# MarSaKi/VLN-BEVBert

Measured on AMD Instinct MI355X. Metric: pretrain_samples_per_sec, higher is better.
Workload: dtype bf16+fp32-residual

## Files before the change

### vln_bevbert_amd/arena.py

```python
import math

import torch

from . import lib
from .lib import ptr, stream


def call(name, *args):
    from . import ops
    return ops.call(name, *args)

CHUNK = 1024
_ZERO_KERNEL = __import__("os").environ.get("BEVBERT_ZERO_KERNEL", "0") == "1"
NO_DECAY = ("bias", "LayerNorm.bias", "LayerNorm.weight")


def _round_up(n, m):
    return (n + m - 1) // m * m


class ParamArena:
    _serial = 0

    def __init__(self, module, device, compute_dtype=torch.float32, groups=()):
        self.device = torch.device(device)
        self.compute_dtype = compute_dtype
        named = [(n, p) for n, p in module.named_parameters()]
        by_name = dict(named)
        in_group = {}
        for gi, g in enumerate(groups):
            for n in g:
                in_group[n] = gi
        layout, seen_groups = [], set()
        for n, p in named:
            if n in in_group:
                gi = in_group[n]
                if gi in seen_groups:
                    continue
                seen_groups.add(gi)
                layout.append(list(groups[gi]))
            else:
                layout.append([n])
        self.slices = {}
        off = 0
        seg_meta = []
        for seg in layout:
            start = off
            decays = set()
            for n in seg:
                k = by_name[n].numel()
                self.slices[n] = (off, k)
                off += k
                decays.add(not any(nd in n for nd in NO_DECAY))
            assert len(decays) == 1, f"group {seg} mixes weight-decay classes"
            off = _round_up(off, CHUNK)
            seg_meta.append((start, off, decays.pop(), seg))
        self.numel = off
        self.n_params = sum(p.numel() for _, p in named)
        dev = self.device
        self.params = torch.zeros(off, dtype=torch.float32, device=dev)
        self.grads = torch.zeros(off, dtype=torch.float32, device=dev)
        self.exp_avg = None
        self.exp_avg_sq = None
        self.shadow = torch.zeros(off, dtype=compute_dtype, device=dev) if compute_dtype != torch.float32 else None
        self._flags_host = torch.zeros(off // CHUNK, dtype=torch.uint8)
        self._seg_of = {}
        for start, end, decay, seg in seg_meta:
            if decay:
                self._flags_host[start // CHUNK:end // CHUNK] |= 1
            for n in seg:
                self._seg_of[n] = (start // CHUNK, end // CHUNK)
        self.flags = self._flags_host.to(dev)
        self.chunk_steps = torch.zeros(off // CHUNK, dtype=torch.int32, device=dev)
        self._touched = set()
        self._flags_dirty = False
        self.publish_grads = True
        self.allreduce_group = None
        self.defer_allreduce = False
        self._cb_queued = False
        self._fresh = []
        self._published = []
        self._param_versions = None
        self.step_count = 0
        self._scalars = torch.zeros(4, dtype=torch.float32, device=dev)
        self._partials = torch.zeros(1024, dtype=torch.float32, device=dev)
        self.named = named
        for n, p in named:
            o, k = self.slices[n]
            view = self.params[o:o + k].view(p.shape)
            view.copy_(p.data.to(dev, torch.float32))
            p.data = view
            p.main_grad = self.grads[o:o + k].view(p.shape)
            p.compute = self.shadow[o:o + k].view(p.shape) if self.shadow is not None else p.data
            p.arena = self
            p.arena_name = n
        self._index = {n: i for i, (n, _) in enumerate(named)}
        self.fold_store = False
        ParamArena._serial += 1
        self.fold_key = ("arena", ParamArena._serial)
        tables = {id(m.weight) for m in module.modules() if isinstance(m, torch.nn.Embedding)}
        self._fold_ranges = []
        for o, k, _ in sorted((*self.slices[n], n) for n, p in named if p.dim() >= 2 and id(p) not in tables):
            if self._fold_ranges and self._fold_ranges[-1][1] == o:
                self._fold_ranges[-1][1] = o + k
            else:
                self._fold_ranges.append([o, o + k])
        self._fold_starts = [a for a, _ in self._fold_ranges]
        self._fold_comp = {}
        self.sync_shadow()
        self._param_versions = sum(p._version for _, p in named)

    def packed(self, names, shape):
        o0, _ = self.slices[names[0]]
        total = 0
        for n in names:
            o, k = self.slices[n]
            assert o == o0 + total, f"{names} are not contiguous in the arena"
            total += k
        assert total == math.prod(shape)
        src = self.shadow if self.shadow is not None else self.params
        return src[o0:o0 + total].view(shape), self.grads[o0:o0 + total].view(shape)

    def touch(self, param):
        n = param.arena_name
        if n not in self._touched:
            self._touched.add(n)
            a, b = self._seg_of[n]
            self._flags_host[a:b] |= 2
            self._flags_dirty = True
        if self.publish_grads:
            self._note_backward_write(param)

    def _note_backward_write(self, param):
        if not self._cb_queued:
            try:
                torch.autograd.Variable._execution_engine.queue_callback(self._publish)
            except RuntimeError:
                return
            self._cb_queued = True
        self._fresh.append(param)

    def _publish(self):
        self._cb_queued = False
        self.sync()
        if self.device.type == "cuda":
            from . import ops
            ops.RT.scratch.reset()
        fresh = self._fresh
        if self.allreduce_group is not None and not self.defer_allreduce:
            import torch.distributed as dist
            dist.all_reduce(self.grads, group=self.allreduce_group)
            self.grads.div_(dist.get_world_size(self.allreduce_group))
            used = torch.zeros(len(self.named), dtype=torch.int32, device=self.grads.device)
            if fresh:
                used[torch.tensor(sorted({self._index[p.arena_name] for p in fresh}), device=used.device)] = 1
            dist.all_reduce(used, op=dist.ReduceOp.MAX, group=self.allreduce_group)
            mine = {id(p) for p in fresh}
            fresh = list(fresh) + [self.named[i][1] for i in used.nonzero().flatten().tolist()
                                   if id(self.named[i][1]) not in mine]
        for p in fresh:
            if p.grad is None:
                p.grad = p.main_grad
                self._published.append(p)
        self._fresh.clear()

    def maybe_lazy_zero(self):
        if self._published and any(p.grad is None for p in self._published):
            for p in self._published:
                p.grad = None
            self._published.clear()
            self.zero_grad()

    def maybe_refresh_shadow(self):
        if self.shadow is None or not self.publish_grads:
            return
        v = 0
        for _, p in self.named:
            v += p._version
        if v != self._param_versions:
            if self._param_versions is not None:
                self.sync_shadow()
            self._param_versions = v

    def sync_shadow(self):
        if self.shadow is not None:
            call("bevbert_cast_f32", ptr(self.params), ptr(self.shadow), self.numel, lib.dtype_code(self.compute_dtype),
                 stream())

    def sync(self):
        if self.device.type == "cuda":
            from . import ops
            ops.WgradStream.flush_all()
            cur = torch.cuda.current_stream(self.device)
            for side in ops.Branches.side_streams():
                if ops.Branches.enabled or side not in ops.WgradStream.streams or ops.WgradStream.dirty:
                    cur.wait_stream(side)
            ops.WgradStream.dirty = False
            ops.WgradStream.release()

    def store_ok(self, sink_ptr, n):
        import bisect
        off, rem = divmod(sink_ptr - self.grads.data_ptr(), 4)
        if rem or off < 0 or off + n > self.numel:
            return False
        i = bisect.bisect_right(self._fold_starts, off) - 1
        return i >= 0 and off + n <= self._fold_ranges[i][1]

    def _arm_fold(self):
        from . import ops
        ops.ReduceQueue.store_ok = self.store_ok if self.fold_store else None
        ops.ReduceQueue.fold_norm = None

    def _name_at(self, sink_ptr):
        off = (sink_ptr - self.grads.data_ptr()) // 4
        return next((n for n, (o, k) in self.slices.items() if o <= off < o + k), f"arena offset {off}")

    def fold_check_zero(self, stores):
        base = self.grads.data_ptr()
        views = [self.grads[(p - base) // 4:(p - base) // 4 + n] for p, n in stores]
        counts = torch.stack([torch.count_nonzero(v) for v in views]).tolist()
        bad = [(self._name_at(p), c) for (p, _), c in zip(stores, counts) if c]
        if bad:
            raise lib.BevBertHipError(
                "store-mode fold: the gradient of " + ", ".join(f"{n} ({c} non-zero elements)" for n, c in bad[:4])
                + " is not zero before the step's fold -- something other than the split-K fold writes it, or the arena "
                "was not zeroed for this step (BEVBERT_FOLD_STORE=0 turns the store mode off)")

    def _fold_complement(self, entry):
        ent = self._fold_comp.get(id(entry))
        if ent is not None and ent[0] is entry:
            return ent[1:]
        if torch.cuda.is_current_stream_capturing():
            raise lib.BevBertHipError("fold-norm complement table missing during graph capture (warm-up steps build it)")
        import numpy as np
        base, recs, pos = self.grads.data_ptr(), [], 0
        for p, n, _ in sorted(entry["norm_jobs"]) + [(base + 4 * self.numel, 0, 0)]:
            o = (p - base) // 4
            for a in range(pos, o, 16384):
                recs.append((base + 4 * a, (min(a + 16384, o) - a) // 4))
            pos = o + n
            assert pos % 4 == 0, "fold sinks are float4-aligned"
        from . import ops
        if entry["nslots"] + len(recs) > ops.ReduceQueue.SLOT_CAPACITY:
            return None
        t = np.zeros(len(recs), dtype=np.dtype([("ptr", "<u8"), ("n4", "<u4"), ("slot", "<u4")]))
        if recs:
            t["ptr"], t["n4"] = zip(*recs)
        t["slot"] = entry["nslots"] + np.arange(len(recs))
        dev = torch.from_numpy(t.view(np.uint8).copy()).to(self.device)
        if len(self._fold_comp) > 64:
            self._fold_comp.clear()
        self._fold_comp[id(entry)] = (entry, dev, len(recs), 16 * int(t["n4"].sum()))
        return dev, len(recs), 16 * int(t["n4"].sum())

    def _clip_from_fold(self, pre_scale, max_norm):
        from . import ops
        rec, ops.ReduceQueue.fold_norm = ops.ReduceQueue.fold_norm, None
        if rec is None or rec["owner"] is not self:
            return False
        entry = rec["entry"]
        comp = self._fold_complement(entry)
        if comp is None:
            return False
        table, ntasks, _ = comp
        slots = ops.ReduceQueue.register_slots(self.device)
        call("bevbert_sumsq_tasks", table.data_ptr(), ntasks, stream())
        call("bevbert_clip_from_slots", ptr(slots), entry["nslots"] + ntasks, pre_scale, max_norm, ptr(self._scalars),
             stream())
        if entry["fresh"] and not torch.cuda.is_current_stream_capturing():
            entry["fresh"] = False
            self._fold_check_norm(entry, slots, pre_scale)
        return True

    def _fold_check_norm(self, entry, slots, pre_scale):
        want = float(torch.linalg.vector_norm(self.grads, dtype=torch.float64)) * pre_scale
        got = float(self._scalars[0])
        if abs(got - want) <= 1e-5 * want or (got == 0.0 and want == 0.0):
            return
        base, culprit = self.grads.data_ptr(), "a range outside the folds"
        for p, n, s0 in entry["norm_jobs"]:
            o = (p - base) // 4
            w = float(self.grads[o:o + n].double().pow(2).sum())
            g = float(slots[s0:s0 + (n // 4 + 4095) // 4096].double().sum())
            if abs(g - w) > 1e-5 * max(w, 1e-30):
                culprit = self._name_at(p)
                break
        raise lib.BevBertHipError(
            f"fused gradient norm {got!r} differs from the arena's {want!r}: the gradient of {culprit} changed after the "
            "step's fold (BEVBERT_FOLD_STORE=0 turns the fused norm off)")

    def backward_done(self):
        self.sync()

    def zero_grad(self, overlap=False):
        self.sync()
        if self.device.type == "cuda":
            from . import ops
            ops.RT.scratch.reset()
            self._arm_fold()
            if overlap:
                if getattr(self, "_zero_stream", None) is None:
                    from .hwqueues import side_stream
                    self._zero_stream = side_stream(self.device)
                self._zero_stream.wait_stream(torch.cuda.current_stream(self.device))
                with torch.cuda.stream(self._zero_stream):
                    if _ZERO_KERNEL:
                        self.grads.zero_()
                    else:
                        call("bevbert_zero", ptr(self.grads), self.grads.numel() * 4, stream())
                self._zero_pending = True
                return
            call("bevbert_zero", ptr(self.grads), self.grads.numel() * 4, stream())
            return
        self.grads.zero_()

    def wait_zero(self):
        if getattr(self, "_zero_pending", False):
            torch.cuda.current_stream(self.device).wait_stream(self._zero_stream)
            self._zero_pending = False

    def load_state_dict_into(self, module, sd, strict=True):
        out = module.load_state_dict(sd, strict=strict)
        self.sync_shadow()
        return out

    def set_lr(self, lr):
        self._scalars[2:3].fill_(float(lr))
        self._lr_set = True

    def upload_flags(self):
        if self._flags_dirty:
            self.flags.copy_(self._flags_host, non_blocking=True)
            self._flags_dirty = False

    def clip_and_step(self, lr=None, betas=(0.9, 0.98), eps=1e-6, weight_decay=0.01, max_norm=5.0, grad_pre_scale=1.0,
                      fused_norm=False):
        self.sync()
        if self.exp_avg is None:
            self.exp_avg = torch.zeros_like(self.params)
            self.exp_avg_sq = torch.zeros_like(self.params)
        if lr is not None:
            self.set_lr(lr)
        elif not getattr(self, "_lr_set", False):
            raise RuntimeError("clip_and_step(lr=None) reads the device-resident learning rate: call set_lr() first "
                               "(the slot starts at 0, which would silently turn AdamW and its weight decay into a no-op)")
        if not torch.cuda.is_current_stream_capturing():
            self.upload_flags()
        self.step_count += 1
        max_norm = float(max_norm if max_norm is not None else -1.0)
        if not (fused_norm and self._clip_from_fold(float(grad_pre_scale), max_norm)):
            call("bevbert_grad_norm_clip", ptr(self.grads), self.numel, float(grad_pre_scale), max_norm,
                 ptr(self._partials), ptr(self._scalars), stream())
        call("bevbert_adamw_step", ptr(self.params), ptr(self.grads), ptr(self.exp_avg), ptr(self.exp_avg_sq),
             ptr(self.shadow), ptr(self.flags), ptr(self.chunk_steps), self.numel, self._scalars[1:].data_ptr(),
             self._scalars[2:].data_ptr(), 0.0, float(betas[0]), float(betas[1]), float(eps), float(weight_decay),
             stream())

    def grad_norm(self):
        return self._scalars[0]
```

### vln_bevbert_amd/csrc/optimizer.hip

```cpp
#include <math.h>
#include <type_traits>

#include "rowops_common.h"

#define ACCUM_U 4
#define ACCUM_SC 4
template <typename T, bool STORE = false>
__device__ __forceinline__ float accum_fold(const T* part_, float* sink_, size_t stride4, size_t n4, int S, size_t first,
                                            size_t step) {
  const BB_GLOBAL T* __restrict__ part = (const BB_GLOBAL T*)part_;
  BB_GLOBAL float* __restrict__ sink = (BB_GLOBAL float*)sink_;
  float sq = 0.f;
  for (size_t i = first; i < n4; i += ACCUM_U * step) {
    size_t idx[ACCUM_U];
    float4 acc[ACCUM_U];
#pragma unroll
    for (int u = 0; u < ACCUM_U; ++u) {
      idx[u] = i + u * step < n4 ? i + u * step : n4 - 1;
      if constexpr (STORE) acc[u] = make_float4(0.f, 0.f, 0.f, 0.f);
      else acc[u] = gld4<float>(sink + idx[u] * 4);
    }
    int s = 0;
    for (; s + ACCUM_SC <= S; s += ACCUM_SC) {
      float4 v[ACCUM_SC][ACCUM_U];
#pragma unroll
      for (int k = 0; k < ACCUM_SC; ++k)
#pragma unroll
        for (int u = 0; u < ACCUM_U; ++u) v[k][u] = gld4<T>(part + ((size_t)(s + k) * stride4 + idx[u]) * 4);
#pragma unroll
      for (int k = 0; k < ACCUM_SC; ++k)
#pragma unroll
        for (int u = 0; u < ACCUM_U; ++u) add4(acc[u], v[k][u]);
    }
    for (; s < S; ++s) {
      float4 v[ACCUM_U];
#pragma unroll
      for (int u = 0; u < ACCUM_U; ++u) v[u] = gld4<T>(part + ((size_t)s * stride4 + idx[u]) * 4);
#pragma unroll
      for (int u = 0; u < ACCUM_U; ++u) add4(acc[u], v[u]);
    }
#pragma unroll
    for (int u = 0; u < ACCUM_U; ++u)
      if (i + u * step < n4) {
        const bb_f4v o = {acc[u].x, acc[u].y, acc[u].z, acc[u].w};
        *reinterpret_cast<BB_GLOBAL bb_f4v*>(sink + idx[u] * 4) = o;
        sq += (acc[u].x * acc[u].x + acc[u].y * acc[u].y) + (acc[u].z * acc[u].z + acc[u].w * acc[u].w);
      }
  }
  return sq;
}

template <typename T>
__global__ __launch_bounds__(256) void accum_partials_kernel(const T* __restrict__ partials, float* __restrict__ sink,
                                                             int S, size_t n4) {
  accum_fold<T>(partials, sink, n4, n4, S, (size_t)blockIdx.x * 256 + threadIdx.x, (size_t)gridDim.x * 256);
}

struct AccumTask {
  const void* partials;
  float* sink;
  unsigned long long n4_total;
  unsigned int off4, n4;
  int S, dtype;
};
#define ACCUM_STORE 0x100
#define ACCUM_NORM 0x200
__device__ __forceinline__ float block_sum_256(float s) {
  __shared__ float sh[4];
  s = wave_sum(s);
  if ((threadIdx.x & 63) == 0) sh[threadIdx.x >> 6] = s;
  __syncthreads();
  return (sh[0] + sh[1]) + (sh[2] + sh[3]);
}
template <typename T, bool STORE>
__device__ __forceinline__ float accum_task(const AccumTask& t) {
  return accum_fold<T, STORE>((const T*)t.partials + (size_t)t.off4 * 4, t.sink, t.n4_total, t.n4, t.S, threadIdx.x, 256);
}
__global__ __launch_bounds__(256) void multi_accum_kernel(const AccumTask* __restrict__ tasks, float* __restrict__ slots,
                                                          unsigned int capacity) {
  const AccumTask t = tasks[blockIdx.x];
  const bool bf16 = (t.dtype & 0xff) == BB_BF16;
  float sq;
  if (t.dtype & ACCUM_STORE) sq = bf16 ? accum_task<bf16_raw, true>(t) : accum_task<float, true>(t);
  else sq = bf16 ? accum_task<bf16_raw, false>(t) : accum_task<float, false>(t);
  const unsigned int slot = (unsigned int)t.dtype >> 12;
  if ((t.dtype & ACCUM_NORM) && slot < capacity) {
    sq = block_sum_256(sq);
    if (threadIdx.x == 0) slots[slot] = sq;
  }
}

__global__ __launch_bounds__(256) void sumsq_kernel(const float* __restrict__ g, size_t n4, float* __restrict__ partials) {
  float s = 0.f;
  for (size_t i = (size_t)blockIdx.x * 256 + threadIdx.x; i < n4; i += (size_t)gridDim.x * 256) {
    const float4 v = *reinterpret_cast<const float4*>(g + i * 4);
    s += (v.x * v.x + v.y * v.y) + (v.z * v.z + v.w * v.w);
  }
  __shared__ float sh[4];
  s = wave_sum(s);
  if ((threadIdx.x & 63) == 0) sh[threadIdx.x >> 6] = s;
  __syncthreads();
  if (threadIdx.x == 0) partials[blockIdx.x] = (sh[0] + sh[1]) + (sh[2] + sh[3]);
}

struct SumsqTask {
  const float* ptr;
  unsigned int n4, slot;
};
__global__ __launch_bounds__(256) void sumsq_tasks_kernel(const SumsqTask* __restrict__ tasks, float* __restrict__ slots,
                                                          unsigned int capacity) {
  const SumsqTask t = tasks[blockIdx.x];
  if (t.slot >= capacity) return;
  const unsigned int n4 = t.n4 < 4096u ? t.n4 : 4096u;
  float s = 0.f;
  if (n4) {
    const BB_GLOBAL float* __restrict__ g = (const BB_GLOBAL float*)t.ptr;
    float4 v[16];
#pragma unroll
    for (int u = 0; u < 16; ++u) {
      const unsigned int i = threadIdx.x + u * 256;
      v[u] = gld4<float>(g + (size_t)(i < n4 ? i : n4 - 1) * 4);
    }
#pragma unroll
    for (int u = 0; u < 16; ++u)
      if (threadIdx.x + u * 256 < n4) s += (v[u].x * v[u].x + v[u].y * v[u].y) + (v[u].z * v[u].z + v[u].w * v[u].w);
  }
  s = block_sum_256(s);
  if (threadIdx.x == 0) slots[t.slot] = s;
}

__global__ void clip_coef_kernel(const float* __restrict__ partials, int n, float pre_scale, float max_norm,
                                 float* __restrict__ scalars) {
  __shared__ double sh[256];
  double s = 0.0;
  for (int i = threadIdx.x; i < n; i += 256) s += (double)partials[i];
  sh[threadIdx.x] = s;
  __syncthreads();
  for (int o = 128; o > 0; o >>= 1) {
    if (threadIdx.x < o) sh[threadIdx.x] += sh[threadIdx.x + o];
    __syncthreads();
  }
  if (threadIdx.x == 0) {
    const float norm = (float)sqrt(sh[0]) * pre_scale;
    float coef = 1.0f;
    if (max_norm > 0.f) {
      coef = max_norm / (norm + 1e-6f);
      coef = coef < 1.0f ? coef : 1.0f;
    }
    scalars[0] = norm;
    scalars[1] = pre_scale * coef;
  }
}

__global__ __launch_bounds__(256) void adamw_kernel(float* __restrict__ p, const float* __restrict__ g,
                                                    float* __restrict__ m, float* __restrict__ v,
                                                    bf16_raw* __restrict__ p_bf16, const uint8_t* __restrict__ flags,
                                                    int* __restrict__ chunk_steps, size_t nchunks,
                                                    const float* __restrict__ gscale_ptr,
                                                    const float* __restrict__ lr_ptr, float lr, float beta1,
                                                    float beta2, float eps, float wd, float log2_beta1,
                                                    float log2_beta2) {
  if (lr_ptr) lr = *lr_ptr;
  const size_t chunk = blockIdx.x;
  if (chunk >= nchunks) return;
  const uint8_t f = flags[chunk];
  if (!(f & 2)) return;
  const int t = chunk_steps[chunk] + 1;
  __syncthreads();
  if (threadIdx.x == 0) chunk_steps[chunk] = t;
  const float bc1 = 1.0f - __builtin_amdgcn_exp2f((float)t * log2_beta1);
  const float bc2 = 1.0f - __builtin_amdgcn_exp2f((float)t * log2_beta2);
  const float step_size = lr * sqrtf(bc2) / bc1;
  const float gs = gscale_ptr ? *gscale_ptr : 1.0f;
  const float decay = (f & 1) ? lr * wd : 0.f;
  const size_t i = chunk * 1024 + threadIdx.x * 4;
  const float4 gg = *reinterpret_cast<const float4*>(g + i);
  float4 pp = *reinterpret_cast<float4*>(p + i);
  float4 mm = *reinterpret_cast<float4*>(m + i);
  float4 vv = *reinterpret_cast<float4*>(v + i);
#define UPD(c)                                                    \
  {                                                               \
    const float gr = gg.c * gs;                                   \
    mm.c = mm.c * beta1 + (1.0f - beta1) * gr;                    \
    vv.c = vv.c * beta2 + (1.0f - beta2) * gr * gr;               \
    pp.c = pp.c - step_size * (mm.c / (sqrtf(vv.c) + eps));       \
    pp.c = pp.c - decay * pp.c;                                   \
  }
  UPD(x) UPD(y) UPD(z) UPD(w)
#undef UPD
  *reinterpret_cast<float4*>(p + i) = pp;
  *reinterpret_cast<float4*>(m + i) = mm;
  *reinterpret_cast<float4*>(v + i) = vv;
  if (p_bf16 != nullptr) st4<bf16_raw>(p_bf16 + i, pp);
}

template <typename TO>
__global__ __launch_bounds__(256) void cast_f32_kernel(const float* __restrict__ src, TO* __restrict__ dst, size_t n4) {
  for (size_t i = (size_t)blockIdx.x * 256 + threadIdx.x; i < n4; i += (size_t)gridDim.x * 256)
    st4<TO>(dst + i * 4, *reinterpret_cast<const float4*>(src + i * 4));
}

BEVBERT_API int bevbert_accum_partials(const void* partials, float* sink, int S, int64_t n, int dtype,
                                       hipStream_t stream) {
  BB_REQUIRE(n % 4 == 0 && S >= 1, "accum_partials: n must be a multiple of 4 and S >= 1");
  if (n == 0) return BB_OK;
  size_t nb = ((size_t)n / 4 + 255) / 256;
  if (nb > 8192) nb = 8192;
  const bool type_ok = bb_with_type(dtype, [&](auto t) {
    using T = decltype(t);
    hipLaunchKernelGGL(accum_partials_kernel<T>, dim3(nb), dim3(256), 0, stream, (const T*)partials, sink, S, (size_t)n / 4);
  });
  if (!type_ok) return bb_dtype_unsupported("accum_partials", dtype);
  BB_CHECK_LAUNCH("accum_partials");
  return BB_OK;
}

BEVBERT_API int bevbert_multi_accum(const void* tasks, int ntasks, hipStream_t stream) {
  static_assert(sizeof(AccumTask) == 40, "AccumTask is part of the C ABI");
  if (ntasks <= 0) return BB_OK;
  BB_REQUIRE(tasks != nullptr, "multi_accum: null task table");
  int capacity = 0;
  float* slots = bb_fold_norm_slots(&capacity);
  hipLaunchKernelGGL(multi_accum_kernel, dim3(ntasks), dim3(256), 0, stream, (const AccumTask*)tasks, slots,
                     (unsigned int)(slots ? capacity : 0));
  BB_CHECK_LAUNCH("multi_accum");
  return BB_OK;
}

BEVBERT_API int bevbert_sumsq_tasks(const void* tasks, int ntasks, hipStream_t stream) {
  static_assert(sizeof(SumsqTask) == 16, "SumsqTask is part of the C ABI");
  if (ntasks <= 0) return BB_OK;
  int capacity = 0;
  float* slots = bb_fold_norm_slots(&capacity);
  BB_REQUIRE(tasks != nullptr && slots != nullptr, "sumsq_tasks: null task table, or no slot array registered");
  hipLaunchKernelGGL(sumsq_tasks_kernel, dim3(ntasks), dim3(256), 0, stream, (const SumsqTask*)tasks, slots,
                     (unsigned int)capacity);
  BB_CHECK_LAUNCH("sumsq_tasks");
  return BB_OK;
}

BEVBERT_API int bevbert_grad_norm_clip(const float* grads, int64_t n, float pre_scale, float max_norm,
                                       float* partials, float* scalars, hipStream_t stream) {
  BB_REQUIRE(n % 4 == 0, "grad_norm_clip: n must be a multiple of 4");
  hipLaunchKernelGGL(sumsq_kernel, dim3(1024), dim3(256), 0, stream, grads, (size_t)n / 4, partials);
  hipLaunchKernelGGL(clip_coef_kernel, dim3(1), dim3(256), 0, stream, partials, 1024, pre_scale, max_norm, scalars);
  BB_CHECK_LAUNCH("grad_norm_clip");
  return BB_OK;
}

BEVBERT_API int bevbert_clip_from_slots(const float* slots, int n, float pre_scale, float max_norm, float* scalars,
                                        hipStream_t stream) {
  BB_REQUIRE(n >= 0 && (slots != nullptr || n == 0) && scalars != nullptr, "clip_from_slots: null pointer or negative count");
  hipLaunchKernelGGL(clip_coef_kernel, dim3(1), dim3(256), 0, stream, slots, n, pre_scale, max_norm, scalars);
  BB_CHECK_LAUNCH("clip_from_slots");
  return BB_OK;
}

BEVBERT_API int bevbert_adamw_step(float* params, const float* grads, float* exp_avg, float* exp_avg_sq,
                                   void* params_bf16, const uint8_t* chunk_flags, int* chunk_steps, int64_t n,
                                   const float* grad_scale_dev, const float* lr_dev, float lr, float beta1,
                                   float beta2, float eps, float weight_decay, hipStream_t stream) {
  BB_REQUIRE(n % 1024 == 0, "adamw_step: arena length must be a multiple of 1024 elements");
  BB_REQUIRE(chunk_steps != nullptr, "adamw_step: per-chunk step counters are required");
  const size_t nchunks = (size_t)n / 1024;
  hipLaunchKernelGGL(adamw_kernel, dim3(nchunks), dim3(256), 0, stream, params, grads, exp_avg, exp_avg_sq,
                     (bf16_raw*)params_bf16, chunk_flags, chunk_steps, nchunks, grad_scale_dev, lr_dev, lr, beta1, beta2, eps,
                     weight_decay, (float)log2((double)beta1), (float)log2((double)beta2));
  BB_CHECK_LAUNCH("adamw_step");
  return BB_OK;
}

BEVBERT_API int bevbert_cast_f32(const float* src, void* dst, int64_t n, int dst_dtype, hipStream_t stream) {
  BB_REQUIRE(n % 4 == 0, "cast_f32: n must be a multiple of 4");
  if (n == 0) return BB_OK;
  size_t nb = ((size_t)n / 4 + 255) / 256;
  if (nb > 8192) nb = 8192;
  const bool type_ok = bb_with_type_of<bf16_raw, _Float16>(dst_dtype, [&](auto t) {
    using T = decltype(t);
    hipLaunchKernelGGL(cast_f32_kernel<T>, dim3(nb), dim3(256), 0, stream, src, (T*)dst, (size_t)n / 4);
  });
  if (!type_ok) {
    bb_set_error("cast_f32: dst dtype %d unsupported", dst_dtype);
    return BB_EUNSUPPORTED;
  }
  BB_CHECK_LAUNCH("cast_f32");
  return BB_OK;
}
```

### vln_bevbert_amd/train.py

```python
import contextlib
import os
import random

import torch
import torch.distributed as dist

from . import capture, ops
from .static_step import GraphedStep, StaticBatch


def warmup_linear_lr(step, base_lr, warmup_steps, total_steps):
    f = step / warmup_steps if step < warmup_steps else max(0, (total_steps - step) / (total_steps - warmup_steps))
    lr = base_lr * f
    return lr if lr > 0 else 1e-8


def load_gemm_tuning():
    import os
    path = os.path.join(os.path.dirname(os.path.abspath(__file__)), "tunableop_results.csv")
    if os.environ.get("BEVBERT_GEMM_TUNING", "1") != "1" or not os.path.exists(path):
        return 0
    try:
        import torch.cuda.tunable as tunable
        tunable.enable(True)
        tunable.tuning_enable(False)
        tunable.record_untuned_enable(False) if hasattr(tunable, "record_untuned_enable") else None
        tunable.set_filename(path + ".unused")
        ok = tunable.read_file(path)
        return len(tunable.get_results()) if ok else 0
    except Exception:
        return 0


class TaskSampler:

    def __init__(self, task_ratio="mlm.5.sap.5.masksem.1", seed=0):
        parts = task_ratio.split(".")
        self.tasks = parts[::2]
        ratios = [int(r) for r in parts[1::2]]
        self.pool = [t for t, r in zip(self.tasks, ratios) for _ in range(r)]
        self.rng = random.Random(seed)

    def next(self):
        return self.rng.choice(self.pool)


class GradReducer:

    def __init__(self, flat_grads, split, group=None, force=False, exchange=None):
        import os
        self.exchange = exchange or os.environ.get("BEVBERT_GRAD_EXCHANGE", "fp32")
        assert self.exchange in ("fp32", "bf16", "bf16_a2a"), self.exchange
        self.flat = flat_grads
        self.split = int(split)
        self.group = group
        self.world = dist.get_world_size(group) if dist.is_available() and dist.is_initialized() else 1
        self.active = self.world > 1 or (force and dist.is_available() and dist.is_initialized())
        self.cuda = flat_grads.is_cuda
        self.stream = None
        if self.cuda and self.active:
            from .hwqueues import side_stream
            self.stream = side_stream(flat_grads.device)
        self.queue_report = None
        self._works = []
        self._phase_a_done = False
        self._done = []
        self.occupied = None
        self.timeline = None

    _settled = {}

    def settle_collective_queue(self):
        if self.queue_report is not None or not (self.cuda and self.active) or \
                os.environ.get("BEVBERT_COLLECTIVE_QUEUE_CHECK", "1") != "1":
            return self.queue_report
        if dist.get_backend(self.group) != "nccl":
            self.queue_report = {"backend": dist.get_backend(self.group), "checked": False}
            return self.queue_report
        settled = GradReducer._settled.get((self.flat.device.index, id(self.group)))
        if settled is not None:
            self.group, self.queue_report = settled
            return self.queue_report
        key = (self.flat.device.index, id(self.group))
        from .hwqueues import steer_stream_pool
        st = steer_stream_pool(self.flat.device, like=self.stream)
        rep = {"steered": st and {"pool": st["pool"], "next": st["next"], "wanted": sum(st["wanted"])},
               "waits_behind_compute": self.collectives_wait_behind_compute()}
        if rep["waits_behind_compute"] and self.group is None:
            st = steer_stream_pool(self.flat.device, like=self.stream)
            self.group = dist.new_group(backend=dist.get_backend())
            rep["own_group"] = {"steered": st and {"pool": st["pool"], "next": st["next"]},
                                "waits_behind_compute": self.collectives_wait_behind_compute()}
        self.queue_report = rep
        GradReducer._settled[key] = (self.group, rep)
        return rep

    def collectives_wait_behind_compute(self, busy_ms=3.0):
        if not (self.cuda and self.active and self.stream is not None):
            return None
        dev = self.flat.device
        main = torch.cuda.current_stream(dev)
        busy = torch.empty(64 << 20, dtype=torch.float32, device=dev)
        t = torch.zeros(256, device=dev)
        dist.all_reduce(t, group=self.group)
        dist.barrier(group=self.group)
        torch.cuda.synchronize(dev)
        from .hwqueues import pick_copy_stream
        issue = pick_copy_stream(dev)
        m1, c1 = torch.cuda.Event(), torch.cuda.Event()
        for _ in range(max(4, int(busy_ms / 0.06))):
            busy.fill_(1.0)
        m1.record(main)
        with torch.cuda.stream(issue):
            dist.all_reduce(t, group=self.group, async_op=True).wait()
            c1.record(issue)
        while not c1.query():
            pass
        waited = torch.tensor([1.0 if m1.query() else 0.0], device=dev)
        torch.cuda.synchronize(dev)
        dist.all_reduce(waited, op=dist.ReduceOp.MAX, group=self.group)
        return bool(waited.item() > 0)

    def drop_pending(self):
        self._works, self._done, self._phase_a_done = [], [], False

    def launch_region(self, lo, hi):
        lo, hi = max(0, int(lo)), min(int(hi), self.flat.numel())
        if self.active and hi > lo:
            self._launch(lo, hi)
            self._done.append((lo, hi))

    def _remaining(self):
        gaps, at = [], 0
        for lo, hi in sorted(self._done):
            if lo > at:
                gaps.append((at, lo))
            at = max(at, hi)
        if at < self.flat.numel():
            gaps.append((at, self.flat.numel()))
        if self.occupied is not None:
            gaps = [(lo, hi) for lo, hi in gaps if self._holds_a_tensor(lo, hi)]
        return gaps

    def _holds_a_tensor(self, lo, hi):
        if self.occupied is None:
            return True
        import bisect
        i = bisect.bisect_right(self._occ_starts, lo) - 1
        return (i >= 0 and self.occupied[i][1] > lo) or (i + 1 < len(self._occ_starts) and self._occ_starts[i + 1] < hi)

    def set_occupied(self, slices):
        self.occupied = sorted((int(o), int(o) + int(k)) for o, k in slices)
        self._occ_starts = [o for o, _ in self.occupied]

    def _exchange_bf16(self, view):
        W, n = self.world, view.numel()
        per = -(-n // W)
        send = torch.zeros(W * per, dtype=torch.bfloat16, device=view.device)
        send[:n].copy_(view)
        if self.exchange == "bf16":
            mine = torch.empty(per, dtype=torch.bfloat16, device=view.device)
            dist.reduce_scatter_tensor(mine, send, op=dist.ReduceOp.SUM, group=self.group)
            dist.all_gather_into_tensor(send, mine, group=self.group)
        else:
            recv = torch.empty_like(send)
            as_wire = (lambda t: t) if view.is_cuda else (lambda t: t.view(torch.uint8))
            dist.all_to_all_single(as_wire(recv), as_wire(send), group=self.group)
            mine = recv.view(W, per).float().sum(0).to(torch.bfloat16)
            dist.all_gather_into_tensor(as_wire(send), as_wire(mine), group=self.group)
        view.copy_(send[:n])

    def _launch(self, lo, hi):
        if hi <= lo:
            return
        view = self.flat[lo:hi]
        if self.cuda:
            ops.WgradStream.flush_all()
        if self.stream is not None:
            self.stream.wait_stream(torch.cuda.current_stream())
            for side in ops.Branches.side_streams():
                if ops.Branches.enabled or side not in ops.WgradStream.streams or ops.WgradStream.dirty:
                    self.stream.wait_stream(side)
            with torch.cuda.stream(self.stream):
                if self.timeline is not None:
                    e0, e1 = torch.cuda.Event(enable_timing=True), torch.cuda.Event(enable_timing=True)
                    e0.record(self.stream)
                    self.timeline.append((lo, hi, e0, e1))
                if self.exchange != "fp32":
                    self._exchange_bf16(view)
                else:
                    self._works.append(dist.all_reduce(view, op=dist.ReduceOp.SUM, group=self.group, async_op=True))
                if self.timeline is not None:
                    if self._works and self.exchange == "fp32":
                        self._works[-1].wait()
                    e1.record(self.stream)
        elif self.exchange != "fp32":
            self._exchange_bf16(view)
        else:
            self._works.append(dist.all_reduce(view, op=dist.ReduceOp.SUM, group=self.group, async_op=True))

    def launch_uncovered(self, lo, hi):
        for a, b in self._remaining():
            a, b = max(a, int(lo)), min(b, int(hi))
            if b > a and self._holds_a_tensor(a, b):
                self.launch_region(a, b)

    def phase_a(self, *_):
        if self.active and not self._phase_a_done:
            self._phase_a_done = True
            self.launch_uncovered(self.split, self.flat.numel())

    def finish(self):
        if self.active:
            for lo, hi in self._remaining():
                self._launch(lo, hi)
            for w in self._works:
                w.wait()
            if self.stream is not None:
                torch.cuda.current_stream().wait_stream(self.stream)
        self._works = []
        self._phase_a_done = False
        self._done = []


def fold_store_allowed(device_type, reducer_active, early_flush, env=None):
    env = os.environ if env is None else env
    return env.get("BEVBERT_FOLD_STORE", "1") == "1" and device_type == "cuda" and not reducer_active and not early_flush


class PretrainTrainer:
    def __init__(self, model, arena, learning_rate=5e-5, warmup_steps=10000, num_train_steps=100000,
                 betas=(0.9, 0.98), weight_decay=0.01, grad_norm=5.0, seed=0, rank=0, world_size=1, overlap=True,
                 force_collectives=False):
        self.model, self.arena = model, arena
        arena.publish_grads = False
        self.lr, self.warmup, self.total = learning_rate, warmup_steps, num_train_steps
        self.betas, self.wd, self.grad_norm = betas, weight_decay, grad_norm
        self.seed, self.rank, self.world = seed, rank, world_size
        self.global_step = 0
        import os
        self.use_graphs = os.environ.get("BEVBERT_GRAPHS", "1") == "1" and arena.device.type == "cuda"
        self.graph_branches = os.environ.get("BEVBERT_GRAPH_BRANCHES", "1") == "1"
        self.overlap_zero = os.environ.get("BEVBERT_OVERLAP_ZERO", "1") == "1" and arena.device.type == "cuda"
        self.graph_error = None
        self._graph_pool = None
        first_map = min(arena.slices[n][0] for n in arena.slices
                        if n.startswith("bert.local_encoder") or n.startswith("bert.global_encoder")
                        or not n.startswith("bert."))
        self.reducer = GradReducer(arena.grads, first_map, force=force_collectives)
        self.reducer.set_occupied(arena.slices.values())
        self.reducer.settle_collective_queue()
        self.overlap = overlap and self.reducer.active
        self.capture_ok = not (self.reducer.active and self.reducer.exchange == "bf16_a2a")
        if self.reducer.active and dist.get_backend(self.reducer.group) != "nccl":
            self.capture_ok = False
        if self.reducer.active:
            self.broadcast_state()
        self.early_flush = os.environ.get("BEVBERT_EARLY_FLUSH", "0") == "1" and arena.device.type == "cuda"
        if self.early_flush and not self.overlap:
            model.bert.lang_encoder.register_forward_hook(self._hook_flush)
        arena.fold_store = fold_store_allowed(arena.device.type, self.reducer.active, self.early_flush)
        if self.overlap:
            self.install_map_layer_hooks()
            model.bert.lang_encoder.register_forward_hook(self._hook_text)
            for k, lo, hi in self.text_layer_regions(model, arena):
                model.bert.lang_encoder.layer[k].register_forward_pre_hook(self._make_layer_hook(lo, hi))

    @staticmethod
    def map_layer_regions(model, arena):
        out = {}
        heads = [(o, o + k) for n, (o, k) in arena.slices.items() if not n.startswith("bert.")]
        if heads:
            lo, hi = min(lo for lo, _ in heads), max(hi for _, hi in heads)
            if not any(n.startswith("bert.") and lo <= o < hi for n, (o, c) in arena.slices.items()):
                out["heads"] = (lo, hi)
        for enc in ("local", "global"):
            mod = getattr(model.bert, f"{enc}_encoder").encoder
            kv = {n for group in mod.arena_groups(f"bert.{enc}_encoder.encoder.") for n in group}
            for k in range(1, len(mod.x_layers)):
                pre = f"bert.{enc}_encoder.encoder.x_layers.{k}."
                own = sorted((o, o + c) for n, (o, c) in arena.slices.items() if n.startswith(pre) and n not in kv)
                if not own:
                    continue
                lo, hi = own[0][0], own[-1][1]
                inside = [n for n, (o, c) in arena.slices.items() if lo <= o < hi and not (n.startswith(pre) and n not in kv)]
                if not inside:
                    out[(enc, k)] = (lo, hi)
        return out

    def install_map_layer_hooks(self):
        regions = self.map_layer_regions(self.model, self.arena)
        self._map_regions = regions
        self._map_uses, self._map_fired, self._heads_sent = {}, {}, False

        def make(enc):
            def hook(k, fired):
                key = (enc, k)
                if not fired:
                    self._map_uses[key] = self._map_uses.get(key, 0) + 1
                    return
                self._map_fired[key] = self._map_fired.get(key, 0) + 1
                if not self._heads_sent and "heads" in regions:
                    self._heads_sent = True
                    self.reducer.launch_region(*regions["heads"])
                if key in regions and self._map_fired[key] == self._map_uses.get(key, 0):
                    self.reducer.launch_region(*regions[key])
            return hook
        for enc in ("local", "global"):
            getattr(self.model.bert, f"{enc}_encoder").encoder.region_hook = make(enc)

    def _reset_map_hooks(self):
        if getattr(self, "_map_regions", None) is not None:
            self._map_uses, self._map_fired, self._heads_sent = {}, {}, False

    @staticmethod
    def text_layer_regions(model, arena, spec=None):
        import os
        if spec is None:
            spec = os.environ.get("BEVBERT_REDUCE_TEXT_LAYERS", "auto")
        n_layers = len(model.bert.lang_encoder.layer)
        if spec.strip() == "auto":
            layers = {round(n_layers / 3), round(2 * n_layers / 3)}
        else:
            layers = {int(x) for x in spec.split(",") if x.strip()}
        hi = max(o + k for n, (o, k) in arena.slices.items() if n.startswith("bert.lang_encoder."))
        out = []
        for k in sorted({x for x in layers if 0 < x < n_layers}, reverse=True):
            lo = min(o for n, (o, _) in arena.slices.items() if n.startswith(f"bert.lang_encoder.layer.{k}."))
            out.append((k, lo, hi))
            hi = lo
        return out

    def _make_layer_hook(self, lo, hi):
        def pre_hook(module, inputs):
            x = inputs[0]
            if torch.is_tensor(x) and x.requires_grad and torch.is_grad_enabled():
                x.register_hook(lambda g: (self.reducer.launch_region(lo, hi), g)[1])
        return pre_hook

    def _hook_flush(self, module, inputs, output):
        if output.requires_grad and torch.is_grad_enabled():
            output.register_hook(lambda g: (ops.WgradStream.flush_all(), g)[1])
        return output

    def _hook_text(self, module, inputs, output):
        if output.requires_grad and torch.is_grad_enabled():
            output.register_hook(lambda g: (self.reducer.phase_a(), g)[1])
        return output

    def broadcast_state(self, src=0):
        if not (dist.is_available() and dist.is_initialized()):
            return
        a = self.arena
        dist.broadcast(a.params, src=src, group=self.reducer.group)
        if a.exp_avg is not None:
            dist.broadcast(a.exp_avg, src=src, group=self.reducer.group)
            dist.broadcast(a.exp_avg_sq, src=src, group=self.reducer.group)
            dist.broadcast(a.chunk_steps, src=src, group=self.reducer.group)
        for b in self.model.buffers():
            dist.broadcast(b, src=src, group=self.reducer.group)
        a.sync_shadow()

    def _step_seed(self):
        return (self.seed + self.rank) * 1000003 + self.global_step

    def forward_backward(self, task, batch):
        self.global_step += 1
        ops.RT.new_step(self._step_seed(), plan_key=self._plan_key(task, batch))
        return self._forward_backward(task, batch)

    @staticmethod
    def _plan_key(task, batch):
        return (task, batch.signature) if isinstance(batch, StaticBatch) else None

    def _forward_backward(self, task, batch):
        self._reset_map_hooks()
        self.arena.zero_grad(overlap=self.overlap_zero)
        try:
            if isinstance(batch, StaticBatch):
                loss = self.model.loss_mean(batch.tensors, task)
            else:
                loss = self.model(batch, task, compute_loss=True).mean()
        finally:
            self.arena.wait_zero()
        if self.reducer is not None and self.reducer.timeline is not None:
            self.backward_start = torch.cuda.Event(enable_timing=True)
            self.backward_start.record()
        if loss.is_cuda and loss.dim() == 0:
            one = self.__dict__.get("_one")
            if one is None or one.dtype != loss.dtype or one.device != loss.device:
                one = self._one = torch.ones((), dtype=loss.dtype, device=loss.device)
            loss.backward(gradient=one)
        else:
            loss.backward()
        self.arena.sync()
        self.reducer.finish()
        return loss.detach()

    def optimizer_step(self, lr=None, fused_norm=False):
        if lr is None:
            lr = warmup_linear_lr(self.global_step, self.lr, self.warmup, self.total)
        self.arena.clip_and_step(lr, self.betas, 1e-6, self.wd, self.grad_norm, grad_pre_scale=1.0 / self.world,
                                 fused_norm=fused_norm)

    def step(self, task, batch):
        if isinstance(batch, StaticBatch) and self.use_graphs and self.capture_ok and batch.capturable and ops.RT.trace is None:
            return self._static_step(task, batch)
        loss = self.forward_backward(task, batch)
        self.optimizer_step(fused_norm=True)
        return loss

    def validate(self, val_loaders, setname="", **kw):
        from .validate import validate
        return validate(self.model, val_loaders, setname, **kw)

    GRAPH_WARMUP = 2

    def _static_step(self, task, sb):
        assert sb.task == task
        self.global_step += 1
        lr = warmup_linear_lr(self.global_step, self.lr, self.warmup, self.total)
        a = self.arena
        if a.exp_avg is None:
            a.exp_avg = torch.zeros_like(a.params)
            a.exp_avg_sq = torch.zeros_like(a.params)
        ops.RT.new_step(self._step_seed(), plan_key=None if (sb.graph is not None and sb.graph.owner is self)
                        else self._plan_key(task, sb))
        a.set_lr(lr)
        gs = sb.graph
        if gs is not None and gs.owner is self:
            a.upload_flags()
            gs.graph.replay()
            return gs.loss.clone()
        if sb.eager_runs < self.GRAPH_WARMUP:
            sb.eager_runs += 1
            with self._capture_stream_layout():
                loss = self._forward_backward(task, sb)
            self.optimizer_step(lr=None, fused_norm=True)
            return loss
        a.upload_flags()
        if self.reducer.active:
            import time
            torch.cuda.synchronize()
            time.sleep(0.3)

        def body():
            ops.RT.new_step(0, write_salt=False, plan_key=self._plan_key(task, sb))
            loss = self._forward_backward(task, sb)
            a.clip_and_step(None, self.betas, 1e-6, self.wd, self.grad_norm, grad_pre_scale=1.0 / self.world,
                            fused_norm=True)
            return loss
        try:
            with self._capture_stream_layout():
                graph, loss = capture.capture(body, self._graph_pool, [self.reducer.stream])
        except capture.CaptureFailed as e:
            import warnings
            self.graph_error = e.message
            self.use_graphs = False
            warnings.warn(f"hipGraph capture of the {task} step failed, continuing with eager steps: {self.graph_error}")
            self.reducer.drop_pending()
            ops.RT.new_step(self._step_seed(), plan_key=self._plan_key(task, sb))
            loss = self._forward_backward(task, sb)
            self.optimizer_step(lr=None, fused_norm=True)
            return loss
        self._graph_pool = graph.pool()
        gs = GraphedStep(graph, loss)
        gs.owner = self
        sb.graph = gs
        graph.replay()
        return loss.clone()

    @contextlib.contextmanager
    def _capture_stream_layout(self):
        branches = ops.Branches.enabled
        ops.Branches.enabled = branches or self.graph_branches
        try:
            yield
        finally:
            ops.Branches.enabled = branches


class ArenaDataParallel(torch.nn.Module):

    def __init__(self, module, process_group=None, compute_dtype=None):
        super().__init__()
        self.module = module
        arena = getattr(module, "arena", None)
        if arena is None:
            dev = next(module.parameters()).device
            arena = module.finalize(dev, compute_dtype or torch.float32)
        self.arena = arena
        if dist.is_available() and dist.is_initialized() and dist.get_world_size(process_group) > 1:
            arena.allreduce_group = process_group if process_group is not None else dist.group.WORLD
            dist.broadcast(arena.params, src=0, group=process_group)
            for b in module.buffers():
                dist.broadcast(b, src=0, group=process_group)
            arena.sync_shadow()

    def forward(self, *args, **kwargs):
        return self.module(*args, **kwargs)

    def no_sync(self):
        import contextlib

        @contextlib.contextmanager
        def ctx():
            old = self.arena.defer_allreduce
            self.arena.defer_allreduce = True
            try:
                yield
            finally:
                self.arena.defer_allreduce = old
        return ctx()


def wrap_model(model, device, local_rank, compute_dtype=None):
    model.to(device)
    if local_rank != -1:
        return ArenaDataParallel(model, compute_dtype=compute_dtype)
    if compute_dtype is not None and getattr(model, "arena", None) is None:
        model.finalize(device, compute_dtype)
    return model
```

Measured before the change: 3787.

## Skip gradient reads and norm work for untouched arena chunks in step

Tracks which parameters were written in the current backward pass and builds a cached per-pass plan that marks untouched chunks as known-zero. The AdamW kernel then skips loading gradients for those chunks via a new flag bit, and the fused grad-norm complement table zeroes out records lying entirely inside zero chunks. The clip-coefficient reduction loop is also unrolled with wider loads. This adds host-side plan building, validation and keyed caching, and relies on every gradient writer calling touch.

```diff
diff --git a/vln_bevbert_amd/arena.py b/vln_bevbert_amd/arena.py
--- a/vln_bevbert_amd/arena.py
+++ b/vln_bevbert_amd/arena.py
@@ -74,6 +74,9 @@
         self.chunk_steps = torch.zeros(off // CHUNK, dtype=torch.int32, device=dev)
         self._touched = set()
         self._flags_dirty = False
+        self._pass_touched = set()
+        self.zero_aware = False
+        self._zero_plans = {}
         self.publish_grads = True
         self.allreduce_group = None
         self.defer_allreduce = False
@@ -128,6 +131,7 @@
             a, b = self._seg_of[n]
             self._flags_host[a:b] |= 2
             self._flags_dirty = True
+        self._pass_touched.add(n)
         if self.publish_grads:
             self._note_backward_write(param)
 
@@ -229,7 +233,7 @@
     def _fold_complement(self, entry):
         ent = self._fold_comp.get(id(entry))
         if ent is not None and ent[0] is entry:
-            return ent[1:]
+            return ent[1:4]
         if torch.cuda.is_current_stream_capturing():
             raise lib.BevBertHipError("fold-norm complement table missing during graph capture (warm-up steps build it)")
         import numpy as np
@@ -250,19 +254,71 @@
         dev = torch.from_numpy(t.view(np.uint8).copy()).to(self.device)
         if len(self._fold_comp) > 64:
             self._fold_comp.clear()
-        self._fold_comp[id(entry)] = (entry, dev, len(recs), 16 * int(t["n4"].sum()))
+        self._fold_comp[id(entry)] = (entry, dev, len(recs), 16 * int(t["n4"].sum()), t)
         return dev, len(recs), 16 * int(t["n4"].sum())
+
+    def _zero_plan(self, entry):
+        touched = frozenset(self._pass_touched)
+        plan = self._zero_plans.get((id(entry), touched))
+        if plan is not None and plan["entry"] is entry:
+            return plan
+        if torch.cuda.is_current_stream_capturing():
+            raise lib.BevBertHipError("zero-aware step plan missing during graph capture (warm-up steps build it)")
+        import numpy as np
+        nchunks = self.numel // CHUNK
+        zero = np.ones(nchunks, dtype=bool)
+        for n in touched:
+            a, b = self._seg_of[n]
+            zero[a:b] = False
+        zero_dev = torch.from_numpy(zero).to(self.device)
+        counts = torch.count_nonzero(self.grads.view(nchunks, CHUNK), dim=1)
+        bad = torch.nonzero((counts > 0) & zero_dev).flatten().tolist()
+        if bad:
+            names = []
+            for c in bad:
+                n = next((n for n, (a, b) in self._seg_of.items()
+                          if a <= c < b and self.slices[n][0] < (c + 1) * CHUNK and c * CHUNK < sum(self.slices[n])),
+                         f"arena chunk {c}")
+                if n not in names:
+                    names.append(n)
+            raise lib.BevBertHipError(
+                "zero-aware step: the gradient of " + ", ".join(names[:4]) + " is not zero although no kernel registered "
+                "a write to it in this backward pass -- a writer that does not call ParamArena.touch "
+                "(BEVBERT_ZERO_AWARE=0 turns the zero-aware tail off)")
+        _, _, ntasks, nbytes, host = self._fold_comp[id(entry)]
+        t = host.copy()
+        if ntasks:
+            o = (t["ptr"].astype(np.int64) - self.grads.data_ptr()) // 4
+            nz = np.concatenate([[0], np.cumsum(~zero)])
+            c0, c1 = o // CHUNK, (o + 4 * t["n4"].astype(np.int64) - 1) // CHUNK
+            inside = nz[c1 + 1] == nz[c0]
+            t["n4"][inside] = 0
+        bits = torch.from_numpy(zero.astype(np.uint8) * 4)
+        plan = {
+            "entry": entry, "touched": touched, "ntasks": ntasks, "bits": bits,
+            "table": torch.from_numpy(t.view(np.uint8).copy()).to(self.device),
+            "flags": (self._flags_host | bits).to(self.device),
+            "zero_records": int((t["n4"] == 0).sum()), "norm_bytes": 16 * int(t["n4"].sum()), "norm_bytes_before": nbytes}
+        self._zero_plans[(id(entry), touched)] = plan
+        return plan
+
+    def zero_plan_adamw_bytes(self, plan):
+        return 4 * CHUNK * int(((plan["bits"] != 0) & ((self._flags_host & 2) != 0)).sum())
 
     def _clip_from_fold(self, pre_scale, max_norm):
         from . import ops
         rec, ops.ReduceQueue.fold_norm = ops.ReduceQueue.fold_norm, None
         if rec is None or rec["owner"] is not self:
-            return False
+            return None
         entry = rec["entry"]
         comp = self._fold_complement(entry)
         if comp is None:
-            return False
+            return None
         table, ntasks, _ = comp
+        flags = self.flags
+        if self.zero_aware:
+            plan = self._zero_plan(entry)
+            table, flags = plan["table"], plan["flags"]
         slots = ops.ReduceQueue.register_slots(self.device)
         call("bevbert_sumsq_tasks", table.data_ptr(), ntasks, stream())
         call("bevbert_clip_from_slots", ptr(slots), entry["nslots"] + ntasks, pre_scale, max_norm, ptr(self._scalars),
@@ -270,7 +326,7 @@
         if entry["fresh"] and not torch.cuda.is_current_stream_capturing():
             entry["fresh"] = False
             self._fold_check_norm(entry, slots, pre_scale)
-        return True
+        return flags
 
     def _fold_check_norm(self, entry, slots, pre_scale):
         want = float(torch.linalg.vector_norm(self.grads, dtype=torch.float64)) * pre_scale
@@ -294,6 +350,7 @@
 
     def zero_grad(self, overlap=False):
         self.sync()
+        self._pass_touched.clear()
         if self.device.type == "cuda":
             from . import ops
             ops.RT.scratch.reset()
@@ -331,6 +388,8 @@
     def upload_flags(self):
         if self._flags_dirty:
             self.flags.copy_(self._flags_host, non_blocking=True)
+            for plan in self._zero_plans.values():
+                plan["flags"].copy_(self._flags_host | plan["bits"])
             self._flags_dirty = False
 
     def clip_and_step(self, lr=None, betas=(0.9, 0.98), eps=1e-6, weight_decay=0.01, max_norm=5.0, grad_pre_scale=1.0,
@@ -348,11 +407,13 @@
             self.upload_flags()
         self.step_count += 1
         max_norm = float(max_norm if max_norm is not None else -1.0)
-        if not (fused_norm and self._clip_from_fold(float(grad_pre_scale), max_norm)):
+        flags = self._clip_from_fold(float(grad_pre_scale), max_norm) if fused_norm else None
+        if flags is None:
             call("bevbert_grad_norm_clip", ptr(self.grads), self.numel, float(grad_pre_scale), max_norm,
                  ptr(self._partials), ptr(self._scalars), stream())
+            flags = self.flags
         call("bevbert_adamw_step", ptr(self.params), ptr(self.grads), ptr(self.exp_avg), ptr(self.exp_avg_sq),
-             ptr(self.shadow), ptr(self.flags), ptr(self.chunk_steps), self.numel, self._scalars[1:].data_ptr(),
+             ptr(self.shadow), ptr(flags), ptr(self.chunk_steps), self.numel, self._scalars[1:].data_ptr(),
              self._scalars[2:].data_ptr(), 0.0, float(betas[0]), float(betas[1]), float(eps), float(weight_decay),
              stream())
 
diff --git a/vln_bevbert_amd/csrc/optimizer.hip b/vln_bevbert_amd/csrc/optimizer.hip
--- a/vln_bevbert_amd/csrc/optimizer.hip
+++ b/vln_bevbert_amd/csrc/optimizer.hip
@@ -129,11 +129,20 @@
   if (threadIdx.x == 0) slots[t.slot] = s;
 }
 
-__global__ void clip_coef_kernel(const float* __restrict__ partials, int n, float pre_scale, float max_norm,
-                                 float* __restrict__ scalars) {
+#define CLIP_U 32
+__global__ __launch_bounds__(256) void clip_coef_kernel(const float* __restrict__ partials_, int n, float pre_scale,
+                                                        float max_norm, float* __restrict__ scalars) {
+  const BB_GLOBAL float* __restrict__ partials = (const BB_GLOBAL float*)partials_;
   __shared__ double sh[256];
   double s = 0.0;
-  for (int i = threadIdx.x; i < n; i += 256) s += (double)partials[i];
+  for (int i = threadIdx.x; i < n; i += CLIP_U * 256) {
+    float v[CLIP_U];
+#pragma unroll
+    for (int u = 0; u < CLIP_U; ++u) v[u] = partials[i + u * 256 < n ? i + u * 256 : n - 1];
+#pragma unroll
+    for (int u = 0; u < CLIP_U; ++u)
+      if (i + u * 256 < n) s += (double)v[u];
+  }
   sh[threadIdx.x] = s;
   __syncthreads();
   for (int o = 128; o > 0; o >>= 1) {
@@ -174,7 +183,8 @@
   const float gs = gscale_ptr ? *gscale_ptr : 1.0f;
   const float decay = (f & 1) ? lr * wd : 0.f;
   const size_t i = chunk * 1024 + threadIdx.x * 4;
-  const float4 gg = *reinterpret_cast<const float4*>(g + i);
+  float4 gg = make_float4(0.f, 0.f, 0.f, 0.f);
+  if (!(f & 4)) gg = *reinterpret_cast<const float4*>(g + i);
   float4 pp = *reinterpret_cast<float4*>(p + i);
   float4 mm = *reinterpret_cast<float4*>(m + i);
   float4 vv = *reinterpret_cast<float4*>(v + i);
diff --git a/vln_bevbert_amd/train.py b/vln_bevbert_amd/train.py
--- a/vln_bevbert_amd/train.py
+++ b/vln_bevbert_amd/train.py
@@ -226,6 +226,11 @@
 def fold_store_allowed(device_type, reducer_active, early_flush, env=None):
     env = os.environ if env is None else env
     return env.get("BEVBERT_FOLD_STORE", "1") == "1" and device_type == "cuda" and not reducer_active and not early_flush
+
+
+def zero_aware_allowed(fold_store, env=None):
+    env = os.environ if env is None else env
+    return bool(fold_store) and env.get("BEVBERT_ZERO_AWARE", "1") == "1"
 
 
 class PretrainTrainer:
@@ -260,6 +265,7 @@
         if self.early_flush and not self.overlap:
             model.bert.lang_encoder.register_forward_hook(self._hook_flush)
         arena.fold_store = fold_store_allowed(arena.device.type, self.reducer.active, self.early_flush)
+        arena.zero_aware = zero_aware_allowed(arena.fold_store)
         if self.overlap:
             self.install_map_layer_hooks()
             model.bert.lang_encoder.register_forward_hook(self._hook_text)
```

Result: no change. 3817 (median of 6 runs) (+0.8%).
